# OneWalkman/EDGE-YOLO

Measured on AMD Instinct MI355X. Metric: images/sec @ 640x640 fp16 (EdgeLine-YOLO detection forward path: backbone + DWT neck + GFLv2 head decode + batched NMS), higher is better.
Workload: dtype f16; 1 GPU; yolo11n-test.yaml (scale n, nc=80) predict path, 640x640, batch 32/GPU, conf 0.25 iou 0.7 max_det 300, random-init weights, default head biases (DENSE NMS regime: mean detections/img 300); regime=dense, global_batch=32, imgsz=640, nc=80

## Files before the change

### edge-yolo_amd/csrc/api.cpp

```cpp
#include <stdarg.h>
#include <stdio.h>
#include <stddef.h>
#include <string.h>
#include "../../include/edgeyolo_hip.h"
#include "tune.h"

static thread_local char g_err[512] = "";

int ey_set_error(int code, const char* fmt, ...) {
  va_list ap;
  va_start(ap, fmt);
  vsnprintf(g_err, sizeof(g_err), fmt, ap);
  va_end(ap);
  return code;
}

extern "C" const char* ey_last_error(void) { return g_err; }
extern "C" int ey_version(void) { return 1; }
extern "C" size_t ey_abi_sizeof(int which) { return which == 0 ? sizeof(ey_conv_desc) : which == 1 ? sizeof(ey_conv_direct_desc) : 0; }

EyTune g_ey_tune;
#define EY_T(f) {#f, offsetof(EyTune, f)}
static const struct { const char* name; size_t off; } k_tunables[] = {
    EY_T(tiles_per_wave), EY_T(mt2_min_m), EY_T(small_m), EY_T(small_wmb), EY_T(halo_min_c), EY_T(ws_lds_kb), EY_T(ws_wg_cu), EY_T(ws_k3_minnt), EY_T(tile_wlds),
    EY_T(tile_s2_minc), EY_T(tile_s2_minm), EY_T(grid_div), EY_T(c3r), EY_T(tile_minwg), EY_T(tile_flat), EY_T(tile_mink), EY_T(pwr_m), EY_T(pwr_frags), EY_T(pw_m),
    EY_T(pw_waves), EY_T(pw_wmb), EY_T(ds_p), EY_T(tz_kmask), EY_T(tz_minpx), EY_T(ds_strip), EY_T(stem_mfma), EY_T(linattn_mfma), EY_T(softattn_mfma), EY_T(areaattn_mfma), EY_T(c3p), EY_T(c3p_min_m), EY_T(c3p_fast), EY_T(c3s), EY_T(c3s_mt4_m), EY_T(c3s_min_work), EY_T(c3s_cfg), EY_T(nms_fast_k), EY_T(nms_mask_wg), EY_T(sppf_min_wg), EY_T(sppf_cv), EY_T(dsb_pair), EY_T(dsb_max_px), EY_T(dsb_rb), EY_T(dsb_fixed), EY_T(dsb_p2), EY_T(stem_pair), EY_T(pw3), EY_T(pw3_min_px), EY_T(pw3_skew), EY_T(scdown), EY_T(scdown_min_px), EY_T(ghost), EY_T(ghost_min_px), EY_T(ghost_sb), EY_T(pwn), EY_T(pwn_max_m), EY_T(pwn_ntw), EY_T(pwc), EY_T(xcd_map), EY_T(nms_mask_k), EY_T(head_lean), EY_T(head_fuse), EY_T(chain_fast)};
static long* tunable(const char* name) {
  if (!name) return nullptr;
  for (const auto& t : k_tunables)
    if (!strcmp(t.name, name)) return (long*)((char*)&g_ey_tune + t.off);
  return nullptr;
}
extern "C" int ey_tune_set(const char* name, long value) {
  long* p = tunable(name);
  if (!p) return ey_set_error(EY_EINVAL, "ey_tune_set: unknown tunable '%s'", name ? name : "(null)");
  *p = value;
  return EY_OK;
}
extern "C" long ey_tune_get(const char* name) {
  const long* p = tunable(name);
  return p ? *p : -1;
}
```

### edge-yolo_amd/csrc/conv_dispatch.inc.h

```cpp
#include "conv_kernels.inc.h"
#include <stdlib.h>
#include "tune.h"

static int conv_nt(int Cout) {
  if (Cout <= 16) return 1;
  if (Cout <= 32) return 2;
  if (Cout <= 64) return 4;
  if (Cout <= 80) return 5;
  if (Cout <= 128) return 8;
  if (Cout % 128 == 0) return 8;
  if (Cout % 80 == 0) return 5;
  if (Cout % 64 == 0) return 4;
  return 8;
}
static int conv_cout_pad(int Cout) { int bn = 16 * conv_nt(Cout); return (Cout + bn - 1) / bn * bn; }
static int conv_kpad(int Cin, int k, int es) { return ey_conv_kpad(k * k * Cin, es); }

#if EY_CONV_PART == 16
extern "C" size_t ey_conv_packed_bytes(int dtype, int Cout, int Cin, int k) {
  return (size_t)conv_cout_pad(Cout) * conv_kpad(Cin, k, dtype == EY_F16 ? 2 : 4) * (dtype == EY_F16 ? 2 : 4);
}

extern "C" int ey_conv_pack_weight(int dtype, int Cout, int Cin, int k, const float* w, void* out, size_t out_bytes) {
  EY_CHECK(dtype == EY_F16 || dtype == EY_F32, "pack: bad dtype %d", dtype);
// ... 148 lines not shown
template <typename T, int NT, int S>
static int halo_launch(ConvP p, int ngroup, hipStream_t st) {
  constexpr int MT = (S == 1) ? 2 : 1, TR = 8, TC = 16 * MT, HR = (TR - 1) * S + 3, HC = (TC - 1) * S + 3;
  const int C = p.srcC[0];
  const size_t lds = ((size_t)16 * NT * p.LSw + (size_t)HR * HC * (C + 8)) * sizeof(T);
  if (!ey_lds_reserve<conv3_halo_kernel<T, NT, S>>(lds)) return ey_set_error(EY_ELAUNCH, "conv: cannot reserve %zu B of LDS for the halo tile", lds);
  const long ntile = (long)p.B * ((p.Wo + TC - 1) / TC) * ((p.Ho + TR - 1) / TR);
  const int ntn = conv_cout_pad(p.Cout) / (16 * NT);
  const int occ = ey_occupancy<conv3_halo_kernel<T, NT, S>>(512, lds);
  const int per_cu = occ < 2 ? occ : 2;
  long gx = (long)256 * per_cu / ((long)ntn * ngroup);
  if (gx < 1) gx = 1;
  if (gx > ntile) gx = ntile;
  hipLaunchKernelGGL((conv3_halo_kernel<T, NT, S>), dim3((unsigned)gx, ntn, ngroup), dim3(512), lds, st, p);
  EY_LAUNCH_CHECK("ey_conv2d(halo)");
  g_last_variant = V_HALO + NT * 10 + S;
  return 1;
}

template <typename T>
static int halo_pick_nt(const ConvP& p, int S) {
  const int MT = (S == 1) ? 2 : 1, TC = 16 * MT, HR = 7 * S + 3, HC = (TC - 1) * S + 3, C = p.srcC[0];
  const size_t halo = (size_t)HR * HC * (C + 8) * sizeof(T);
  return conv_widest_nt(conv_nt(p.Cout), 8, [&](int nt) { return halo + (size_t)16 * nt * p.Kpad * sizeof(T) <= 158 * 1024; });
}

template <typename T>
static int dispatch_halo(ConvP p, int ngroup, hipStream_t st) {
  if (p.k != 3 || p.nsrc != 1 || p.srcUp[0] || p.srcC[0] > 64 || p.srcC[0] < tune().halo_min_c) return 0;
  const int S = p.stride;
  {
    const int MT = (S == 1) ? 2 : 1, HR = 7 * S + 3, HC = (16 * MT - 1) * S + 3;
    if ((long)HR * HC * (p.srcC[0] >> 3) > 512L * 10) return 0;
  }
  if (!conv_src_views<T>(p, ngroup)) return 0;
  p.NTpack = conv_nt(p.Cout);
  p.LSw = p.Kpad;
  const int nt = halo_pick_nt<T>(p, S);
  return conv_pick<1, 2, 4, 5, 8>(nt, [&](auto NT) { return conv_pick<1, 2>(S, [&](auto S_) { return halo_launch<T, NT, S_>(p, ngroup, st); }); });
}

template <typename T, int NT, int S>
static int tile_launch(ConvP p, int ngroup, hipStream_t st) {
  constexpr int TR = 8, TC = (S == 1) ? 32 : 16, HR = (TR - 1) * S + 3, HC = (TC - 1) * S + 3, LROW = (S == 1) ? HC : 2 * ((HC + 1) / 2);
  const bool wlds = tune().tile_wlds == 1 || (tune().tile_wlds == 2 && S == 1);
  const size_t lds = ((size_t)HR * LROW + (wlds ? 9 * 16 * NT : 0)) * 40 * sizeof(T);
  p.tTR = TR; p.tTC = TC;
  if (S == 1 && tune().tile_flat) conv_flat_tile(p.Ho, p.Wo, p.tTR, p.tTC);
  const long tiles = (long)p.B * ((p.Wo + p.tTC - 1) / p.tTC) * ((p.Ho + p.tTR - 1) / p.tTR);
  const dim3 grid((unsigned)tiles, (unsigned)(conv_cout_pad(p.Cout) / (16 * NT)), (unsigned)ngroup);
  p.xcd = (int)((tune().xcd_map >> 4) & 1) && grid.y == 1 && grid.z == 1;
  (void)ey_lds_reserve<conv3_tile_kernel<T, NT, S, true>>(100 * 1024);
  if (wlds) hipLaunchKernelGGL((conv3_tile_kernel<T, NT, S, true>), grid, dim3(256), lds, st, p);
  else hipLaunchKernelGGL((conv3_tile_kernel<T, NT, S, false>), grid, dim3(256), lds, st, p);
  EY_LAUNCH_CHECK("ey_conv2d(tile)");
  g_last_variant = V_TILE + NT * 10 + S;
  return 1;
}

template <typename T>
static int dispatch_tile(ConvP p, int ngroup, hipStream_t st) {
  if constexpr (sizeof(T) != 2) return 0;
  else {
    if (p.k != 3 || p.nsrc != 1 || p.srcUp[0] || 9L * p.srcC[0] < tune().tile_mink) return 0;
    if (p.stride == 2 && (p.srcC[0] < tune().tile_s2_minc || (long)p.B * p.Ho * p.Wo < tune().tile_s2_minm)) return 0;
    const int ntp = conv_nt(p.Cout);
    int nt = ntp % 4 == 0 ? 4 : ntp == 2 ? 2 : ntp == 1 ? 1 : 0;
    if (!nt) return 0;
    if (p.stride == 1 && tune().tile_minwg > 0) {
      const long tiles = (long)p.B * (((long)p.Ho * p.Wo + 239) / 240);
      while (nt > 1 && tiles * (conv_cout_pad(p.Cout) / (16 * nt)) * ngroup < tune().tile_minwg) nt >>= 1;
    }
    if (!conv_src_views<T>(p, ngroup) || !conv_weights_fit<T>(p)) return 0;
    p.NTpack = ntp;
    return conv_pick<1, 2, 4>(nt, [&](auto NT) { return conv_pick<1, 2>(p.stride, [&](auto S) { return tile_launch<T, NT, S>(p, ngroup, st); }); });
  }
}

template <int NT, int S>
static int c3r_launch(const ConvP& p, int ngroup, hipStream_t st) {
  int occ = ey_occupancy<conv3r_kernel<NT, S>>(256, 0);
  if (occ > 4) occ = 4;
  const long ntile = (long)p.B * p.Ho * ((p.Wo + 15) / 16);
  if (ntile >= (1L << 31)) return 0;
  long gx = (long)256 * occ / ngroup / tune().grid_div;
  if (gx > (ntile + 3) / 4) gx = (ntile + 3) / 4;
  if (gx < 1) gx = 1;
  hipLaunchKernelGGL((conv3r_kernel<NT, S>), dim3((unsigned)gx, 1, (unsigned)ngroup), dim3(256), 0, st, p);
  EY_LAUNCH_CHECK("ey_conv2d(c3r)");
  g_last_variant = V_C3R + NT * 10 + S;
  return 1;
}

template <typename T>
static int dispatch_c3r(ConvP p, int ngroup, hipStream_t st) {
  if constexpr (sizeof(T) != 2) return 0;
  else {
    if (!tune().c3r || p.k != 3 || p.nsrc != 1 || p.srcUp[0] || p.srcC[0] != 16 || (p.srcCs[0] * 2) % 8) return 0;
    if (p.stride != 2 && tune().c3r < 2) return 0;
    const int ntp = conv_nt(p.Cout);
    if (ntp > 2 || conv_cout_pad(p.Cout) != 16 * ntp) return 0;
    if (!conv_src_views<T>(p, ngroup)) return 0;
    p.NTpack = ntp;
    return conv_pick<1, 2>(ntp, [&](auto NT) { return conv_pick<1, 2>(p.stride, [&](auto S) { return c3r_launch<NT, S>(p, ngroup, st); }); });
  }
}

template <int NT>
static int c3p_launch(ConvP p, hipStream_t st) {
  p.tTR = 8; p.tTC = 32;
  conv_flat_tile(p.Ho, p.Wo, p.tTR, p.tTC);
  const long tiles = (long)p.B * ((p.Wo + p.tTC - 1) / p.tTC) * ((p.Ho + p.tTR - 1) / p.tTR);
  if (tiles >= (1L << 30)) return 0;
  const int ny = conv_cout_pad(p.Cout) / (16 * NT);
  const size_t lds = ((size_t)9 * 16 * NT + 340) * 80 * 2;
  if (!ey_lds_reserve<conv3p_kernel<NT, true>>(lds) || !ey_lds_reserve<conv3p_kernel<NT, false>>(lds)) return 0;
  long gx = 256 / ny;
  if (gx < 1) gx = 1;
  if (gx > tiles) gx = tiles;
  const long ybytes = (((long)p.B * p.Ho * p.Wo - 1) * p.yCs + p.Cout) * 2L;
  const bool fast = tune().c3p_fast && p.bias && p.act == EY_ACT_SILU && p.out_scale == 1.f && !p.res && !p.addz && p.vec_store == 2 && p.Cout % (16 * NT) == 0 &&
                    ybytes < (1L << 31);
  p.srcBytes[1] = fast ? (unsigned)ybytes : 0u;
  const dim3 gg((unsigned)gx, (unsigned)ny, 1);
  if (fast) hipLaunchKernelGGL((conv3p_kernel<NT, true>), gg, dim3(256), lds, st, p);
  else hipLaunchKernelGGL((conv3p_kernel<NT, false>), gg, dim3(256), lds, st, p);
  EY_LAUNCH_CHECK("ey_conv2d(c3p)");
  g_last_variant = V_C3P + NT * 10 + (fast ? 1 : 0);
  return 1;
}

template <typename T>
static int dispatch_c3p(ConvP p, int ngroup, hipStream_t st) {
  if constexpr (sizeof(T) != 2) return 0;
  else {
    if (!tune().c3p || p.k != 3 || p.stride != 1 || p.nsrc != 1 || p.srcUp[0] || ngroup != 1 || p.srcC[0] != 64) return 0;
    const int ntp = conv_nt(p.Cout);
    if (ntp % 4 != 0 || conv_cout_pad(p.Cout) % 64) return 0;
    const long M = (long)p.B * p.Ho * p.Wo;
    if (tune().c3p < 2 && M < tune().c3p_min_m) return 0;
    if (!conv_src_views<T>(p, ngroup) || !conv_weights_fit<T>(p)) return 0;
    p.NTpack = ntp;
    return c3p_launch<4>(p, st);
  }
}

template <int NT, int MT, int UPT, int S, int NB>
static int c3s_launch(ConvP p, hipStream_t st) {
  const size_t lds = (size_t)16 * NT * p.LSw * 2;
  if (!ey_lds_reserve<conv3s_kernel<NT, MT, UPT, S, NB>>(lds)) return 0;
  const long M = (long)p.B * p.Ho * p.Wo;
  p.ntile = (M + 16 * MT - 1) / (16 * MT);
  const int ny = conv_cout_pad(p.Cout) / (16 * NT);
  long gx = 256 / ny;
  if (gx < 1) gx = 1;
  if (gx * 8 > p.ntile) gx = (p.ntile + 7) / 8;
  p.xcd = (int)((tune().xcd_map >> 3) & 1) && (ny == 1 || gx % 8 == 0);
  hipLaunchKernelGGL((conv3s_kernel<NT, MT, UPT, S, NB>), dim3((unsigned)gx, (unsigned)ny, 1), dim3(512), lds, st, p);
  EY_LAUNCH_CHECK("ey_conv2d(c3s)");
  g_last_variant = V_C3S + NT * 100 + MT * 10 + (NB == 9 ? 5 : 0) + S;
  return 1;
}

template <typename T>
static int dispatch_c3s(ConvP p, int ngroup, hipStream_t st) {
  if constexpr (sizeof(T) != 2) return 0;
  else {
    if (!tune().c3s || p.k != 3 || p.nsrc != 1 || p.srcUp[0] || ngroup != 1) return 0;
    const int Cin = p.srcC[0];
    if (Cin != 64 && Cin != 128 && Cin != 256) return 0;
    const int ntp = conv_nt(p.Cout);
    if (conv_cout_pad(p.Cout) != p.Cout && conv_cout_pad(p.Cout) / 16 != ntp) return 0;
    const int nt = conv_widest_nt(ntp, 4, [&](int n) { return (size_t)16 * n * p.Kpad * 2 <= 156 * 1024; });
    if (!nt) return 0;
    if (!conv_src_views<T>(p, ngroup) || !conv_weights_fit<T>(p)) return 0;
    p.NTpack = ntp;
    p.LSw = p.Kpad;
    const long M = (long)p.B * p.Ho * p.Wo;
    const long work = M * (conv_cout_pad(p.Cout) / (16 * nt));
    if (tune().c3s < 2 && (p.stride != 2 || work < tune().c3s_min_work)) return 0;
    long cfg = tune().c3s_cfg;
    if (!cfg) cfg = (nt == 4 && M >= tune().c3s_mt4_m) ? 43 : 23;
    const auto go = [&](auto NT, auto MT) {
      return conv_pick<1, 2, 4>(Cin / 64, [&](auto UPT) { return conv_pick<1, 2>(p.stride, [&](auto S) { return c3s_launch<NT, MT, UPT, S, 3>(p, st); }); });
    };
    if (nt == 4 && cfg == 43) return go(std::integral_constant<int, 4>(), std::integral_constant<int, 4>());
    return conv_pick<1, 2, 4>(nt, [&](auto NT) { return go(NT, std::integral_constant<int, 2>()); });
  }
}

template <typename T, int NT>
static int small_launch(ConvP p, int ngroup, hipStream_t st) {
  constexpr int BATCH = sizeof(T) == 2 ? 8 : 4;
  const long M = (long)p.B * p.Ho * p.Wo;
  p.ntile = (M + 15) / 16;
  p.ntn = conv_cout_pad(p.Cout) / (16 * NT);
  const long waves = p.ntile * p.ntn;
  hipLaunchKernelGGL((conv_small_kernel<T, NT, BATCH>), dim3((unsigned)((waves + 3) / 4), 1, ngroup), dim3(256), 0, st, p);
  EY_LAUNCH_CHECK("ey_conv2d(small)");
  g_last_variant = V_SMALL + NT * 10 + BATCH;
  return 1;
}

static int small_pick_nt(int Cout, int es) {
  return conv_widest_nt(conv_nt(Cout), es == 2 ? 5 : 2, [](int) { return true; });
}

static bool small_ok(int Cout, int Kpad, int k, long M, int es) {
  if (k != 1 || M >= tune().small_m) return false;
  return ((M + 15) / 16) * (long)conv_cout_pad(Cout) * Kpad * es <= (tune().small_wmb << 20);
}

template <typename T>
static int dispatch_small(ConvP p, int ngroup, hipStream_t st) {
  const long M = (long)p.B * p.Ho * p.Wo;
  if (!small_ok(p.Cout, p.Kpad, p.k, M, sizeof(T))) return 0;
  if (!conv_src_views<T>(p, ngroup)) return 0;
  conv_count_k(p);
  if (p.nsrc == 1) { p.srcC[1] = p.srcC[0]; p.srcCs[1] = p.srcCs[0]; p.srcUp[1] = p.srcUp[0]; p.src[1] = p.src[0]; }
  p.NTpack = conv_nt(p.Cout);
  const int nt = small_pick_nt(p.Cout, sizeof(T));
  const auto go = [&](auto NT) { return small_launch<T, NT>(p, ngroup, st); };
  if constexpr (sizeof(T) == 2) return conv_pick<1, 2, 4, 5>(nt, go);
  else return conv_pick<1, 2>(nt, go);
}

static int pw_pick_nt(int Cout, long mtiles, int es) {
  const int ntp = conv_nt(Cout), rows = conv_cout_pad(Cout) / 16;
  const int opts[5] = {8, 5, 4, 2, 1};
  int pick = 0;
  for (int i = 0; i < 5; ++i) {
    const int nt = opts[i];
    if (nt > ntp || ntp % nt || (es == 4 && nt > 4)) continue;
    pick = nt;
    if (mtiles * (rows / nt) >= tune().pw_waves || nt <= 2) break;
  }
  return pick;
}

template <typename T, int NT, int TWO, int GEO>
static int pw_launch(const ConvP& p, hipStream_t st) {
  constexpr int BATCH = (sizeof(T) == 2 ? (NT <= 2 ? 8 : NT <= 5 ? 4 : 2) : (NT <= 2 ? 4 : 2));
  const dim3 grid((unsigned)((p.ntile + 3) / 4), (unsigned)(conv_cout_pad(p.Cout) / (16 * NT)), 1);
  hipLaunchKernelGGL((conv_pw_kernel<T, NT, BATCH, TWO != 0, GEO != 0>), grid, dim3(256), 0, st, p);
  EY_LAUNCH_CHECK("ey_conv2d(pw)");
  g_last_variant = V_PW + NT * 10 + (TWO ? 2 : 1);
  return 1;
}

template <typename T>
static int dispatch_pw(ConvP p, int ngroup, hipStream_t st) {
  const long M = (long)p.B * p.Ho * p.Wo;
  if (p.k != 1 || p.stride != 1 || ngroup != 1 || M >= tune().pw_m) return 0;
  if (((M + 15) / 16) * (long)conv_cout_pad(p.Cout) * p.Kpad * (long)sizeof(T) > (tune().pw_wmb << 20)) return 0;
  if (!conv_weights_fit<T>(p) || !conv_src_views<T>(p, ngroup)) return 0;
  p.ntile = (M + 15) / 16;
  p.NTpack = conv_nt(p.Cout);
  const int nt = pw_pick_nt(p.Cout, p.ntile, sizeof(T));
  const bool two = p.nsrc == 2, geo = p.addz != nullptr || p.srcUp[0] || (two && p.srcUp[1]);
  const auto go = [&](auto NT) {
    return conv_pick<0, 1>(two, [&](auto TWO) { return conv_pick<0, 1>(geo, [&](auto GEO) { return pw_launch<T, NT, TWO, GEO>(p, st); }); });
  };
  if constexpr (sizeof(T) == 2) return conv_pick<1, 2, 4, 5, 8>(nt, go);
  else return conv_pick<1, 2, 4>(nt, go);
}

template <typename T, int NT, int KS, int TWO, int GEO>
static int pwr_launch(const ConvP& p, hipStream_t st) {
  int occ = ey_occupancy<conv_pwr_kernel<T, NT, KS, TWO != 0, GEO != 0>>(256, 0);
  if (occ > 4) occ = 4;
  const unsigned ny = (unsigned)(conv_cout_pad(p.Cout) / (16 * NT));
  long gx = (long)256 * occ / ny / tune().grid_div;
  const long need = (p.ntile + 3) / 4;
  if (gx > need) gx = need;
  if (gx < 1) gx = 1;
  hipLaunchKernelGGL((conv_pwr_kernel<T, NT, KS, TWO != 0, GEO != 0>), dim3((unsigned)gx, ny, 1), dim3(256), 0, st, p);
  EY_LAUNCH_CHECK("ey_conv2d(pwr)");
  g_last_variant = V_PWR + NT * 10 + KS;
  return 1;
}

template <typename T>
static int dispatch_pwr(ConvP p, int ngroup, hipStream_t st) {
  if constexpr (sizeof(T) != 2) return 0;
  else {
    const long M = (long)p.B * p.Ho * p.Wo;
    if (p.k != 1 || p.stride != 1 || ngroup != 1 || M < tune().pwr_m || !p.vec_store || M >= (1L << 27)) return 0;
    const int ntp = conv_nt(p.Cout);
    if (conv_cout_pad(p.Cout) != 16 * ntp) return 0;
    if (p.Cout != 16 * ntp) return 0;
    const int ks = (p.srcC[0] + 31) / 32 + (p.nsrc == 2 ? (p.srcC[1] + 31) / 32 : 0);
    if (ks * ntp > tune().pwr_frags || ks > 4) return 0;
    if (!conv_src_views<T>(p, ngroup)) return 0;
    p.ntile = (M + 15) / 16;
    p.NTpack = ntp;
    const bool two = p.nsrc == 2, geo = p.addz != nullptr || p.srcUp[0] || (two && p.srcUp[1]);
    return conv_pick<1, 2, 4, 5, 8>(ntp, [&](auto NT) {
      return conv_pick<1, 2, 3, 4>(ks, [&](auto KS) {
        if constexpr (KS == 4 && NT > 4) return 0;
        else return conv_pick<0, 1>(two, [&](auto TWO) { return conv_pick<0, 1>(geo, [&](auto GEO) { return pwr_launch<T, NT, KS, TWO, GEO>(p, st); }); });
      });
    });
  }
}

template <int KS, int NTW>
static int pwn_launch(ConvP p, hipStream_t st) {
  int units = KS * 4;
  while ((units & 3) != 2) ++units;
  p.LSw = units * 8;
  const size_t lds = (size_t)64 * p.LSw * 2;
  if (!ey_lds_reserve<conv_pwn_kernel<KS, NTW>>(lds)) return ey_set_error(EY_ELAUNCH, "conv(pwn): cannot reserve %zu B of LDS", lds);
  const long M = (long)p.B * p.Ho * p.Wo;
// ... 215 lines not shown
```

### edge-yolo_amd/csrc/conv_kernels.inc.h

```cpp
#include "common.h"
#include <type_traits>

struct ConvP {
  int B, H, W, Ho, Wo, Cout, k, stride, pad, act, nsrc;
  const void* src[2];
  int srcC[2], srcCs[2], srcUp[2];
  const void* w;
  const float* bias;
  void* y;
  int yCs;
  const void* res;
  int resCs;
  float out_scale;
  const void* addz;
  int addzCs, Hz, Wz;
  float zsy, zsx;
  long srcG, yG;
  long wG;
  int wGmax;
  int Kpad;
  int nchunks;
  unsigned srcBytes[2];
  int Ctot, nsteps;
  int NTpack;
// ... 871 lines not shown
    hyx[u] = (hy << 16) | hx;
  }
  Vec8<T> hv[NHV];
  auto issue_halo = [&](int tile) {
    const int b = tile / tiles_img, trem = tile - b * tiles_img;
    const int iy0 = (trem / tilesX) * tTR - 1, ix0 = (trem % tilesX) * tTC - 1;
#pragma unroll
    for (int u = 0; u < NHV; ++u) {
      const int iy = iy0 + (hyx[u] >> 16), ix = ix0 + (hyx[u] & 0xFFFF);
      const bool ok = (hlo[u] >= 0) & (iy >= 0) & (iy < p.H) & (ix >= 0) & (ix < p.W);
      BufLoad8<T>::load(hv[u], rs, ok ? (unsigned)((((b * p.H + iy) * p.W + ix) * p.srcCs[0] + (threadIdx.x & 7) * 8) * 2) : EY_OOB, 0);
    }
  };
  int bbase[MT], prow[MT], pcol[MT];
#pragma unroll
  for (int mt = 0; mt < MT; ++mt) {
    const int q = wave * 64 + mt * 16 + r;
    const bool qv = q < tTR * tTC;
    prow[mt] = qv ? (int)(((float)q + 0.5f) * inv_tc) : 0;
    pcol[mt] = qv ? q - prow[mt] * tTC : 0;
    bbase[mt] = (prow[mt] * hHC + pcol[mt]) * CP + 8 * g;
    if (!qv) prow[mt] = 1 << 20;
  }
  const T* wlane = wl + r * CP + 8 * g;
  const int BNp = 16 * p.NTpack;
  const int ch0 = (n_base / BNp) * BNp + g * 4 * p.NTpack + 4 * ((n_base % BNp) >> 4);

  f32x4 acc[2][MT][NT];
  float bz[4 * NT];
  unsigned yoff[MT];
  unsigned oh[2 * NT];
  __amdgpu_buffer_rsrc_t ry = ey_rsrc(p.y, p.srcBytes[1]);
  if constexpr (FAST) {
#pragma unroll
    for (int q = 0; q < NT; ++q) {
      const f32x4 bv = *reinterpret_cast<const f32x4*>(p.bias + ch0 + 4 * q);
#pragma unroll
      for (int j = 0; j < 4; ++j) bz[4 * q + j] = bv[j];
    }
#pragma unroll
    for (int mt = 0; mt < MT; ++mt) yoff[mt] = EY_OOB;
  }
  auto set_yoff = [&](int t) {
    const int b = t / tiles_img, trem = t - b * tiles_img;
#pragma unroll
    for (int mt = 0; mt < MT; ++mt) {
      const int oy = (trem / tilesX) * tTR + prow[mt], ox = (trem % tilesX) * tTC + pcol[mt];
      yoff[mt] = (oy < p.Ho && ox < p.Wo) ? (unsigned)(((((long)b * p.Ho + oy) * p.Wo + ox) * p.yCs + ch0) * 2) : EY_OOB;
    }
  };
  auto quarter = [&](const f32x4 (&src)[MT][NT], int mt, int q) {
    float v[4];
#pragma unroll
    for (int j = 0; j < 4; ++j) {
      v[j] = src[mt][q][j] + bz[4 * q + j];
      v[j] = v[j] * ey_sigmoid(v[j]);
    }
    const f16x4 h = {(f16)v[0], (f16)v[1], (f16)v[2], (f16)v[3]};
    const uint2 u = __builtin_bit_cast(uint2, h);
    oh[2 * q] = u.x;
    oh[2 * q + 1] = u.y;
    if (q == NT - 1) {
#pragma unroll
      for (int c = 0; c < NT / 2; ++c) {
        const u32x4 d = {oh[4 * c], oh[4 * c + 1], oh[4 * c + 2], oh[4 * c + 3]};
        __builtin_amdgcn_raw_buffer_store_b128(d, ry, (int)yoff[mt], 16 * c, 0);
      }
    }
  };
  auto tile_body = [&](auto cur_c, int tile) {
    constexpr int CUR = decltype(cur_c)::value;
    ey_lds_barrier();
#pragma unroll
    for (int u = 0; u < NHV; ++u)
      if (hlo[u] >= 0) hv[u].store(hl + hlo[u]);
    ey_lds_barrier();
    if (tile + gridDim.x < ntiles) issue_halo(tile + gridDim.x);
#pragma unroll
    for (int mt = 0; mt < MT; ++mt)
#pragma unroll
      for (int nt = 0; nt < NT; ++nt) acc[CUR][mt][nt] = (f32x4)0.f;
    Vec8<T> af[2][NT], bf[2][MT];
    auto ld_step = [&](int k, Vec8<T> (&a)[NT], Vec8<T> (&bq)[MT]) {
      const int tap = k >> 1, ks = k & 1;
      const int toff = ((tap / 3) * hHC + tap % 3) * CP + ks * 32;
#pragma unroll
      for (int nt = 0; nt < NT; ++nt) a[nt].load(wlane + (tap * 16 * NT + nt * 16) * CP + ks * 32);
#pragma unroll
      for (int mt = 0; mt < MT; ++mt) bq[mt].load(hl + bbase[mt] + toff);
    };
    ld_step(0, af[0], bf[0]);
#pragma unroll
    for (int k = 0; k < 18; ++k) {
      if (k < 17) ld_step(k + 1, af[(k + 1) & 1], bf[(k + 1) & 1]);
      __builtin_amdgcn_sched_barrier(0);
#pragma unroll
      for (int mt = 0; mt < MT; ++mt)
#pragma unroll
        for (int nt = 0; nt < NT; ++nt) acc[CUR][mt][nt] = mma16(af[k & 1][nt], bf[k & 1][mt], acc[CUR][mt][nt]);
      if constexpr (FAST) {
        if (k < MT * NT) quarter(acc[1 - CUR], k / NT, k % NT);
#pragma unroll
        for (int i = 0; i < MT * NT; ++i) {
          __builtin_amdgcn_sched_group_barrier(0x008, 1, 0);
          __builtin_amdgcn_sched_group_barrier(0x002, 2, 0);
        }
      }
      __builtin_amdgcn_sched_barrier(0);
    }
    if constexpr (FAST) {
      set_yoff(tile);
    } else {
      const int b = tile / tiles_img, trem = tile - b * tiles_img;
#pragma unroll
      for (int mt = 0; mt < MT; ++mt) {
        const int oy = (trem / tilesX) * tTR + prow[mt], ox = (trem % tilesX) * tTC + pcol[mt];
        if (oy < p.Ho && ox < p.Wo) conv_epilogue<T, NT>(p, acc[CUR][mt], ((long)b * p.Ho + oy) * p.Wo + ox, b, oy, ox, ch0, 0);
      }
    }
  };

  int tile = blockIdx.x;
  if (tile < ntiles) issue_halo(tile);
  int last = -1;
  while (tile < ntiles) {
    tile_body(std::integral_constant<int, 0>{}, tile);
    last = 0;
    tile += gridDim.x;
    if (tile >= ntiles) break;
    tile_body(std::integral_constant<int, 1>{}, tile);
    last = 1;
    tile += gridDim.x;
  }
  if constexpr (FAST) {
    if (last == 0) {
#pragma unroll
      for (int mt = 0; mt < MT; ++mt)
#pragma unroll
        for (int q = 0; q < NT; ++q) quarter(acc[0], mt, q);
    } else if (last == 1) {
#pragma unroll
      for (int mt = 0; mt < MT; ++mt)
#pragma unroll
        for (int q = 0; q < NT; ++q) quarter(acc[1], mt, q);
    }
  }
}

template <int NT, int MT, int UPT, int S, int NB>
__global__ __launch_bounds__(512, 2) void conv3s_kernel(ConvP p) {
  typedef f16 T;
  extern __shared__ __attribute__((aligned(16))) char smem[];
  T* wl = reinterpret_cast<T*>(smem);
  constexpr int BN = 16 * NT, CIN = 64 * UPT, NU = 9 * UPT;
  const int lane = threadIdx.x & 63, wave = threadIdx.x >> 6;
  const int r = lane & 15, g = lane >> 4;
  const int n_base = blockIdx.y * BN;
  {
    const T* wg = (const T*)p.w + (long)n_base * p.Kpad;
    const int nvec = BN * (p.Kpad >> 3);
    for (int v0 = threadIdx.x; v0 < nvec; v0 += 512 * 8) {
      Vec8<T> w[8];
#pragma unroll
      for (int u = 0; u < 8; ++u)
        if (v0 + u * 512 < nvec) w[u].load(wg + (long)(v0 + u * 512) * 8);
#pragma unroll
      for (int u = 0; u < 8; ++u)
        if (v0 + u * 512 < nvec) w[u].store(wl + (v0 + u * 512) * 8);
    }
  }
  __syncthreads();
  const long M = (long)p.B * p.Ho * p.Wo;
  const int hw = p.Ho * p.Wo;
  const T* wlane = wl + r * p.LSw + 8 * g;
  const int BNp = 16 * p.NTpack;
  const int ch0 = (n_base / BNp) * BNp + g * 4 * p.NTpack + 4 * ((n_base % BNp) >> 4);
  const __amdgpu_buffer_rsrc_t rs = ey_rsrc(p.src[0], p.srcBytes[0]);
  const int Cs = p.srcCs[0], rowB = p.W * Cs * 2;

  struct Desc { int base[MT]; unsigned vm[MT]; };
  auto setup = [&](long tile, Desc& d) {
#pragma unroll
    for (int mt = 0; mt < MT; ++mt) {
      const long m = tile * (16 * MT) + mt * 16 + r;
      const bool pv = m < M;
      const long mm = pv ? m : 0;
      const int b = (int)(mm / hw), rem = (int)(mm - (long)b * hw);
      const int oy = rem / p.Wo, ox = rem - oy * p.Wo;
      const int iy0 = oy * S - 1, ix0 = ox * S - 1;
      d.base[mt] = ((b * p.H + iy0) * p.W + ix0) * Cs * 2 + 16 * g;
      unsigned vm = 0u;
#pragma unroll
      for (int t = 0; t < 9; ++t) {
        const int iy = iy0 + t / 3, ix = ix0 + t % 3;
        vm |= (pv && iy >= 0 && iy < p.H && ix >= 0 && ix < p.W) ? (1u << t) : 0u;
      }
      d.vm[mt] = vm;
    }
  };
  Vec8<T> bq[NB][MT][2];
  auto issue = [&](const Desc& d, int u, Vec8<T> (&bf)[MT][2]) {
    const int tap = u / UPT, c0 = (u - tap * UPT) * 64;
    const int ky = tap / 3, kx = tap - 3 * ky;
    const int toff = ky * rowB + (kx * Cs + c0) * 2;
#pragma unroll
    for (int mt = 0; mt < MT; ++mt) {
      const unsigned vo = ((d.vm[mt] >> tap) & 1u) ? (unsigned)(d.base[mt] + toff) : EY_OOB;
      BufLoad8<T>::load(bf[mt][0], rs, vo, 0);
      BufLoad8<T>::load(bf[mt][1], rs, vo, 64);
    }
  };
  f32x4 acc[MT][NT];
  auto compute = [&](int u, const Vec8<T> (&bf)[MT][2]) {
    const T* wk = wlane + u * 64;
#pragma unroll
    for (int ks = 0; ks < 2; ++ks) {
      Vec8<T> af[NT];
#pragma unroll
      for (int nt = 0; nt < NT; ++nt) af[nt].load(wk + nt * 16 * p.LSw + ks * 32);
#pragma unroll
      for (int mt = 0; mt < MT; ++mt)
#pragma unroll
        for (int nt = 0; nt < NT; ++nt) acc[mt][nt] = mma16(af[nt], bf[mt][ks], acc[mt][nt]);
    }
  };

  const long lb = p.xcd ? ey_xcd_block(blockIdx.x, gridDim.x) : blockIdx.x;
  const long tpw = (p.ntile + gridDim.x - 1) / gridDim.x, tend = min(p.ntile, (lb + 1) * tpw);
  long tile = lb * tpw + wave;
  if (tile >= tend) return;
  Desc cur, nxt;
  setup(tile, cur);
#pragma unroll
  for (int j = 0; j < NB - 1; ++j) issue(cur, j, bq[j]);
  while (true) {
    const long ntl = tile + 8;
    const bool more = ntl < tend;
    if (more) setup(ntl, nxt);
#pragma unroll
    for (int mt = 0; mt < MT; ++mt)
#pragma unroll
      for (int nt = 0; nt < NT; ++nt) acc[mt][nt] = (f32x4)0.f;
#pragma unroll 1
    for (int u = 0; u < NU; u += NB) {
#pragma unroll
      for (int j = 0; j < NB; ++j) {
        const int uu = u + j + NB - 1;
        if (uu < NU) issue(cur, uu, bq[(j + NB - 1) % NB]);
        else if (more) issue(nxt, uu - NU, bq[(j + NB - 1) % NB]);
        compute(u + j, bq[j]);
      }
    }
#pragma unroll
    for (int mt = 0; mt < MT; ++mt) {
      const long m = tile * (16 * MT) + mt * 16 + r;
      if (m < M) {
        const int b = (int)(m / hw), rem = (int)(m - (long)b * hw);
        const int oy = rem / p.Wo;
        conv_epilogue<T, NT>(p, acc[mt], m, b, oy, rem - oy * p.Wo, ch0, 0);
      }
    }
    if (!more) break;
    cur = nxt;
    tile = ntl;
  }
}

typedef f16 f16x4v __attribute__((ext_vector_type(4)));
template <int NT, int S>
__global__ __launch_bounds__(256) void conv3r_kernel(ConvP p) {
  typedef f16 T;
  const int lane = threadIdx.x & 63, r = lane & 15, g = lane >> 4;
  const int grp = blockIdx.z;
  const __amdgpu_buffer_rsrc_t rs = ey_rsrc((const T*)p.src[0] + (long)grp * p.srcG, p.srcBytes[0]);
  f16x4v af[9][NT];
  {
    const T* wg = (const T*)p.w + (long)min(grp, p.wGmax) * p.wG;
#pragma unroll
    for (int tap = 0; tap < 9; ++tap)
#pragma unroll
      for (int nt = 0; nt < NT; ++nt) af[tap][nt] = *reinterpret_cast<const f16x4v*>(wg + (long)(nt * 16 + r) * p.Kpad + tap * 16 + 4 * g);
  }
  const int tilesX = (p.Wo + 15) >> 4;
  const int ntile = p.B * p.Ho * tilesX;
  const int nwave = gridDim.x * 4, wid = blockIdx.x * 4 + (threadIdx.x >> 6);
  const int per = (ntile + nwave - 1) / nwave;
  int tile = wid * per;
  const int tend = min(ntile, tile + per);
  if (tile >= tend) return;
  const int ch0 = g * 4 * NT;
  int row0 = tile / tilesX;
  int ntx = tile - row0 * tilesX, nb = row0 / p.Ho, noy = row0 - nb * p.Ho;
  auto issue = [&](f16x4v (&bq)[9], int& b, int& oy, int& ox) {
    b = nb; oy = noy; ox = ntx * 16 + r;
    const int ix0 = ox * S - 1;
#pragma unroll
    for (int ky = 0; ky < 3; ++ky) {
      const int iy = oy * S - 1 + ky;
      const bool yok = iy >= 0 && iy < p.H && ox < p.Wo;
      const int rowoff = ((b * p.H + iy) * p.W + ix0) * p.srcCs[0] + 4 * g;
#pragma unroll
      for (int kx = 0; kx < 3; ++kx) {
        const int ix = ix0 + kx;
        const unsigned off = (yok && ix >= 0 && ix < p.W) ? (unsigned)((rowoff + kx * p.srcCs[0]) * 2) : EY_OOB;
        typedef unsigned u32x2 __attribute__((ext_vector_type(2)));
        const u32x2 t = __builtin_amdgcn_raw_buffer_load_b64(rs, (int)off, 0, 0);
        bq[ky * 3 + kx] = __builtin_bit_cast(f16x4v, t);
      }
    }
    if (++ntx == tilesX) { ntx = 0; if (++noy == p.Ho) { noy = 0; ++nb; } }
  };
  f16x4v cur[9], nxt[9];
  int b = 0, oy = 0, ox = 0, b2 = 0, oy2 = 0, ox2 = 0;
  issue(cur, b, oy, ox);
  for (; tile < tend; ++tile) {
    if (tile + 1 < tend) issue(nxt, b2, oy2, ox2);
    f32x4 acc[NT];
#pragma unroll
    for (int nt = 0; nt < NT; ++nt) acc[nt] = (f32x4)0.f;
#pragma unroll
    for (int tap = 0; tap < 9; ++tap)
#pragma unroll
      for (int nt = 0; nt < NT; ++nt) acc[nt] = __builtin_amdgcn_mfma_f32_16x16x16f16(af[tap][nt], cur[tap], acc[nt], 0, 0, 0);
    if (ox < p.Wo) conv_epilogue<T, NT>(p, acc, ((long)b * p.Ho + oy) * p.Wo + ox, b, oy, ox, ch0, grp);
#pragma unroll
    for (int tap = 0; tap < 9; ++tap) cur[tap] = nxt[tap];
    b = b2; oy = oy2; ox = ox2;
  }
}

template <int KS, int NTW>
__global__ __launch_bounds__(512) void conv_pwn_kernel(ConvP p) {
  typedef f16 T;
  constexpr int MB = 4, PX = 16 * MB;
  extern __shared__ __attribute__((aligned(16))) char smem[];
  T* s_px = reinterpret_cast<T*>(smem);
  const int tid = threadIdx.x, lane = tid & 63, wave = tid >> 6, r = lane & 15, g = lane >> 4;
  const int KP = p.LSw, KV = KS * 4;
  const int M = p.B * p.Ho * p.Wo, m0 = blockIdx.x * PX;
  const int blk = NTW == 2 ? 2 * blockIdx.y + (wave >> 2) : blockIdx.y;
  const int nt0 = NTW == 2 ? 2 * (wave & 3) : wave;
  Vec8<T> af[KS][NTW];
  {
    const T* wr = (const T*)p.w + (long)(blk * 128 + nt0 * 16 + r) * p.Kpad + 8 * g;
#pragma unroll
    for (int ks = 0; ks < KS; ++ks)
#pragma unroll
      for (int nt = 0; nt < NTW; ++nt) af[ks][nt].load(wr + (long)nt * 16 * p.Kpad + ks * 32);
  }
  {
    const __amdgpu_buffer_rsrc_t rs0 = ey_rsrc(p.src[0], p.srcBytes[0]);
    const __amdgpu_buffer_rsrc_t rs1 = p.nsrc == 2 ? ey_rsrc(p.src[1], p.srcBytes[1]) : rs0;
    const int C0 = p.srcC[0], hw = p.Ho * p.Wo;
    const bool geo = p.srcUp[0] || (p.nsrc == 2 && p.srcUp[1]);
    constexpr int NV = PX * KS * 4, U = (NV + 511) / 512;
    Vec8<T> t[U];
#pragma unroll
    for (int u = 0; u < U; ++u) {
      const int v = tid + u * 512, px = v / KV, c = (v - px * KV) * 8, m = m0 + px;
      const bool second = c >= C0;
      const int s = second ? 1 : 0, cc = second ? c - C0 : c;
      unsigned off = EY_OOB;
      if (v < NV && m < M) {
        if (geo) {
          const int b = m / hw, rem = m - b * hw, oy = rem / p.Wo, ox = rem - oy * p.Wo, up = p.srcUp[s];
          off = (unsigned)(((((b * (p.H >> up)) + (oy >> up)) * (p.W >> up) + (ox >> up)) * p.srcCs[s] + cc) * 2);
        } else {
          off = (unsigned)((m * p.srcCs[s] + cc) * 2);
        }
      }
      BufLoad8<T>::load(t[u], second ? rs1 : rs0, off);
    }
#pragma unroll
    for (int u = 0; u < U; ++u) {
      const int v = tid + u * 512, px = v / KV, c = (v - px * KV) * 8;
      if (v < NV) t[u].store(s_px + px * KP + c);
    }
  }
  __syncthreads();
  f32x4 acc[MB][NTW];
#pragma unroll
  for (int mb = 0; mb < MB; ++mb)
#pragma unroll
    for (int nt = 0; nt < NTW; ++nt) acc[mb][nt] = (f32x4)0.f;
  const T* bp = s_px + r * KP + 8 * g;
#pragma unroll
  for (int ks = 0; ks < KS; ++ks) {
// ... 432 lines not shown
```

### edge-yolo_amd/csrc/tune.h

```cpp
#pragma once
struct EyTune {
  long tiles_per_wave = 0;
  long mt2_min_m = 300000;
  long small_m = 100000;
  long small_wmb = 48;
  long halo_min_c = 48;
  long ws_lds_kb = 76;
  long ws_wg_cu = 2;
  long ws_k3_minnt = 0;
  long tile_wlds = 1;
  long tile_s2_minc = 64;
  long tile_s2_minm = 40000;
  long grid_div = 1;
  long c3p = 1;
  long c3p_min_m = 40000;
  long c3p_fast = 1;
  long c3s = 1;
  long c3s_mt4_m = 100000;
  long c3s_min_work = 20000;
  long c3s_cfg = 0;
  long c3r = 1;
  long tile_minwg = 400;
  long tile_flat = 1;
  long tile_mink = 0;
  long pwr_m = 110000;
  long pwr_frags = 24;
  long pw_m = 110000;
  long pw_waves = 3072;
  long pw_wmb = 64;
  long xcd_map = 31;
  long pwc = 1;
  long pwn = 1;
  long pwn_max_m = 110000;
  long pwn_ntw = 0;
  long ds_p = 0;
  long tz_kmask = 168;
  long tz_minpx = 100000;
  long ds_strip = 1;
  long dsb_pair = 1;
  long dsb_max_px = 300000;
  long dsb_rb = 0;
  long dsb_p2 = 0;
  long dsb_fixed = 100;
  long stem_pair = 1;
  long pw3 = 1;
  long pw3_skew = 8;
  long pw3_min_px = 100000;
  long scdown = 1;
  long scdown_min_px = 0;
  long ghost = 1;
  long ghost_min_px = 0;
  long ghost_sb = 0;
  long stem_mfma = 1;
  long linattn_mfma = 1;
  long softattn_mfma = 1;
  long areaattn_mfma = 1;
  long sppf_min_wg = 128;
  long sppf_cv = 0;
  long nms_mask_wg = 0;
  long nms_mask_k = 1536;
  long head_fuse = 2;
  long head_lean = 1;
  long chain_fast = 1;
  long nms_fast_k = 2048;
};
extern EyTune g_ey_tune;
static inline const EyTune& tune() { return g_ey_tune; }
```

Measured before the change: 29340 images/s.

## Overlap c3s weight staging with first input prefetch via direct global-to-LDS loads

```diff
diff --git a/edge-yolo_amd/csrc/api.cpp b/edge-yolo_amd/csrc/api.cpp
--- a/edge-yolo_amd/csrc/api.cpp
+++ b/edge-yolo_amd/csrc/api.cpp
@@ -24,7 +24,7 @@
 static const struct { const char* name; size_t off; } k_tunables[] = {
     EY_T(tiles_per_wave), EY_T(mt2_min_m), EY_T(small_m), EY_T(small_wmb), EY_T(halo_min_c), EY_T(ws_lds_kb), EY_T(ws_wg_cu), EY_T(ws_k3_minnt), EY_T(tile_wlds),
     EY_T(tile_s2_minc), EY_T(tile_s2_minm), EY_T(grid_div), EY_T(c3r), EY_T(tile_minwg), EY_T(tile_flat), EY_T(tile_mink), EY_T(pwr_m), EY_T(pwr_frags), EY_T(pw_m),
-    EY_T(pw_waves), EY_T(pw_wmb), EY_T(ds_p), EY_T(tz_kmask), EY_T(tz_minpx), EY_T(ds_strip), EY_T(stem_mfma), EY_T(linattn_mfma), EY_T(softattn_mfma), EY_T(areaattn_mfma), EY_T(c3p), EY_T(c3p_min_m), EY_T(c3p_fast), EY_T(c3s), EY_T(c3s_mt4_m), EY_T(c3s_min_work), EY_T(c3s_cfg), EY_T(nms_fast_k), EY_T(nms_mask_wg), EY_T(sppf_min_wg), EY_T(sppf_cv), EY_T(dsb_pair), EY_T(dsb_max_px), EY_T(dsb_rb), EY_T(dsb_fixed), EY_T(dsb_p2), EY_T(stem_pair), EY_T(pw3), EY_T(pw3_min_px), EY_T(pw3_skew), EY_T(scdown), EY_T(scdown_min_px), EY_T(ghost), EY_T(ghost_min_px), EY_T(ghost_sb), EY_T(pwn), EY_T(pwn_max_m), EY_T(pwn_ntw), EY_T(pwc), EY_T(xcd_map), EY_T(nms_mask_k), EY_T(head_lean), EY_T(head_fuse), EY_T(chain_fast)};
+    EY_T(pw_waves), EY_T(pw_wmb), EY_T(ds_p), EY_T(tz_kmask), EY_T(tz_minpx), EY_T(ds_strip), EY_T(stem_mfma), EY_T(linattn_mfma), EY_T(softattn_mfma), EY_T(areaattn_mfma), EY_T(c3p), EY_T(c3p_min_m), EY_T(c3p_fast), EY_T(c3s), EY_T(c3s_mt4_m), EY_T(c3s_min_work), EY_T(c3s_cfg), EY_T(c3s_wg_tiles), EY_T(nms_fast_k), EY_T(nms_mask_wg), EY_T(sppf_min_wg), EY_T(sppf_cv), EY_T(dsb_pair), EY_T(dsb_max_px), EY_T(dsb_rb), EY_T(dsb_fixed), EY_T(dsb_p2), EY_T(stem_pair), EY_T(pw3), EY_T(pw3_min_px), EY_T(pw3_skew), EY_T(scdown), EY_T(scdown_min_px), EY_T(ghost), EY_T(ghost_min_px), EY_T(ghost_sb), EY_T(pwn), EY_T(pwn_max_m), EY_T(pwn_ntw), EY_T(pwc), EY_T(xcd_map), EY_T(nms_mask_k), EY_T(head_lean), EY_T(head_fuse), EY_T(chain_fast)};
 static long* tunable(const char* name) {
   if (!name) return nullptr;
   for (const auto& t : k_tunables)
diff --git a/edge-yolo_amd/csrc/conv_dispatch.inc.h b/edge-yolo_amd/csrc/conv_dispatch.inc.h
--- a/edge-yolo_amd/csrc/conv_dispatch.inc.h
+++ b/edge-yolo_amd/csrc/conv_dispatch.inc.h
@@ -324,13 +324,18 @@
   const long M = (long)p.B * p.Ho * p.Wo;
   p.ntile = (M + 16 * MT - 1) / (16 * MT);
   const int ny = conv_cout_pad(p.Cout) / (16 * NT);
-  long gx = 256 / ny;
+  long gx = 256 / ny / std::max(1L, tune().grid_div);
   if (gx < 1) gx = 1;
-  if (gx * 8 > p.ntile) gx = (p.ntile + 7) / 8;
+  const long mint = std::min(8L, std::max(1L, tune().c3s_wg_tiles));
+  if (gx * mint > p.ntile) {
+    const long full = gx;
+    gx = (p.ntile + mint - 1) / mint;
+    if (ny > 1 && full % 8 == 0) gx = std::min(full, (gx + 7) / 8 * 8);
+  }
   p.xcd = (int)((tune().xcd_map >> 3) & 1) && (ny == 1 || gx % 8 == 0);
   hipLaunchKernelGGL((conv3s_kernel<NT, MT, UPT, S, NB>), dim3((unsigned)gx, (unsigned)ny, 1), dim3(512), lds, st, p);
   EY_LAUNCH_CHECK("ey_conv2d(c3s)");
-  g_last_variant = V_C3S + NT * 100 + MT * 10 + (NB == 9 ? 5 : 0) + S;
+  g_last_variant = V_C3S + NT * 100 + MT * 10 + S;
   return 1;
 }
 
diff --git a/edge-yolo_amd/csrc/conv_kernels.inc.h b/edge-yolo_amd/csrc/conv_kernels.inc.h
--- a/edge-yolo_amd/csrc/conv_kernels.inc.h
+++ b/edge-yolo_amd/csrc/conv_kernels.inc.h
@@ -1047,24 +1047,11 @@
   typedef f16 T;
   extern __shared__ __attribute__((aligned(16))) char smem[];
   T* wl = reinterpret_cast<T*>(smem);
-  constexpr int BN = 16 * NT, CIN = 64 * UPT, NU = 9 * UPT;
+  constexpr int BN = 16 * NT, NU = 9 * UPT;
+  static_assert(NU % NB == 0, "the ring has to divide a tile's units");
   const int lane = threadIdx.x & 63, wave = threadIdx.x >> 6;
   const int r = lane & 15, g = lane >> 4;
   const int n_base = blockIdx.y * BN;
-  {
-    const T* wg = (const T*)p.w + (long)n_base * p.Kpad;
-    const int nvec = BN * (p.Kpad >> 3);
-    for (int v0 = threadIdx.x; v0 < nvec; v0 += 512 * 8) {
-      Vec8<T> w[8];
-#pragma unroll
-      for (int u = 0; u < 8; ++u)
-        if (v0 + u * 512 < nvec) w[u].load(wg + (long)(v0 + u * 512) * 8);
-#pragma unroll
-      for (int u = 0; u < 8; ++u)
-        if (v0 + u * 512 < nvec) w[u].store(wl + (v0 + u * 512) * 8);
-    }
-  }
-  __syncthreads();
   const long M = (long)p.B * p.Ho * p.Wo;
   const int hw = p.Ho * p.Wo;
   const T* wlane = wl + r * p.LSw + 8 * g;
@@ -1121,13 +1108,26 @@
   };
 
   const long lb = p.xcd ? ey_xcd_block(blockIdx.x, gridDim.x) : blockIdx.x;
-  const long tpw = (p.ntile + gridDim.x - 1) / gridDim.x, tend = min(p.ntile, (lb + 1) * tpw);
-  long tile = lb * tpw + wave;
-  if (tile >= tend) return;
+  const long tend = (lb + 1) * p.ntile / gridDim.x;
+  long tile = lb * p.ntile / gridDim.x + wave;
+  const bool work = tile < tend;
   Desc cur, nxt;
-  setup(tile, cur);
-#pragma unroll
-  for (int j = 0; j < NB - 1; ++j) issue(cur, j, bq[j]);
+  if (work) {
+    setup(tile, cur);
+#pragma unroll
+    for (int j = 0; j < NB - 1; ++j) issue(cur, j, bq[j]);
+  }
+  {
+    typedef __attribute__((address_space(1))) const void* gptr_t;
+    typedef __attribute__((address_space(3))) void* lptr_t;
+    const T* wg = (const T*)p.w + (long)n_base * p.Kpad;
+    const int nvec = BN * (p.Kpad >> 3);
+    const int wv0 = __builtin_amdgcn_readfirstlane(wave) * 64;
+    for (int v0 = wv0; v0 < nvec; v0 += 512)
+      if (v0 + lane < nvec) __builtin_amdgcn_global_load_lds((gptr_t)(wg + (long)(v0 + lane) * 8), (lptr_t)(wl + (long)v0 * 8), 16, 0, 0);
+  }
+  __syncthreads();
+  if (!work) return;
   while (true) {
     const long ntl = tile + 8;
     const bool more = ntl < tend;
diff --git a/edge-yolo_amd/csrc/tune.h b/edge-yolo_amd/csrc/tune.h
--- a/edge-yolo_amd/csrc/tune.h
+++ b/edge-yolo_amd/csrc/tune.h
@@ -18,6 +18,7 @@
   long c3s = 1;
   long c3s_mt4_m = 100000;
   long c3s_min_work = 20000;
+  long c3s_wg_tiles = 1;
   long c3s_cfg = 0;
   long c3r = 1;
   long tile_minwg = 400;
```

Measured after the change: 29330 images/s. Within noise of the previous version (-0.0%).
